# stattlab/azplugins

Hardware: AMD Instinct MI355X
Metric: particle-steps/sec, PerturbedLennardJones pair force (higher is better)
Workload: dtype f64

## Files before the change

### azplugins_amd/_lib.py

```python

import ctypes as C
import os

_HERE = os.path.dirname(os.path.abspath(__file__))
LIB_PATH = os.environ.get("AZP_LIB_PATH", os.path.join(_HERE, "libazp.so"))
CSRC = os.path.join(_HERE, "csrc")


class AzpError(RuntimeError):
    pass


class Box(C.Structure):
    _fields_ = [("L", C.c_double * 3), ("tilt", C.c_double * 3), ("periodic", C.c_int32 * 3), ("_pad", C.c_int32)]


class PairArgs(C.Structure):
    _fields_ = [
        ("d_force", C.c_void_p),
        ("d_virial", C.c_void_p),
        ("virial_pitch", C.c_uint64),
        ("N", C.c_uint32),
        ("n_max", C.c_uint32),
        ("d_pos", C.c_void_p),
# ... 607 lines not shown
    "azp_colloid_params_make": (None, [_D] * 4 + [_VP]),
    "azp_colloid_params_unpack": (None, [_VP] + [_PD] * 4),
    "azp_tpm_params_make": (None, [_D] * 5 + [C.c_int, _VP]),
    "azp_tpm_params_unpack": (None, [_VP] + [_PD] * 5 + [_PI]),
    "azp_dw_params_make": (None, [_D] * 4 + [_VP]),
    "azp_dw_params_unpack": (None, [_VP] + [_PD] * 4),
    "azp_quartic_params_make": (None, [_D] * 8 + [_VP]),
    "azp_quartic_params_unpack": (None, [_VP] + [_PD] * 8),
    "azp_table_pack": (C.c_int, [_D, _D, _VP, _VP, C.c_uint32, C.c_int, _VP]),
    "azp_pair_forces_table": (C.c_int, [C.POINTER(PairArgs), _VP, _VP]),
    "azp_pair_forces_planned_table": (C.c_int, [_VP, C.POINTER(PairArgs), _VP, _VP]),
    "azp_bond_forces_table": (C.c_int, [C.POINTER(BondArgs), _VP, _VP, _VP]),
    "azp_pair_forces_perturbed_lennard_jones": (C.c_int, [C.POINTER(PairArgs), _VP, _VP]),
    "azp_pair_forces_hertz": (C.c_int, [C.POINTER(PairArgs), _VP, _VP]),
    "azp_pair_forces_expanded_yukawa": (C.c_int, [C.POINTER(PairArgs), _VP, _VP]),
    "azp_pair_forces_colloid": (C.c_int, [C.POINTER(PairArgs), _VP, _VP]),
    "azp_pair_forces_dpd_conservative": (C.c_int, [C.POINTER(PairArgs), _VP, _VP]),
    "azp_pair_plan_create": (C.c_int, [C.POINTER(_VP)]),
    "azp_pair_plan_destroy": (None, [_VP]),
    "azp_pair_plan_build": (C.c_int, [_VP, C.POINTER(PairArgs), _VP]),
    "azp_pair_plan_build_from_cells": (C.c_int, [_VP, C.POINTER(NlistArgs), C.POINTER(PairArgs), _VP]),
    "azp_pair_plan_set_bank_order": (C.c_int, [_VP, C.c_int]),
    "azp_pair_plan_set_balance": (C.c_int, [_VP, C.c_int]),
    "azp_pair_plan_tile_stage": (C.c_int, [_VP, C.POINTER(C.c_uint32), C.c_uint32]),
    "azp_pair_plan_query": (C.c_int, [_VP, C.POINTER(PlanInfo)]),
    "azp_pair_plan_phase_chunks": (C.c_int, [_VP, C.POINTER(C.c_float)]),
    "azp_pair_plan_shells": (C.c_uint32, []),
    "azp_pair_plan_shells_for": (C.c_uint32, [_D, C.c_int, _D]),
    "azp_pair_plan_row_batches": (C.c_int, [_VP, C.POINTER(C.c_uint32), C.c_uint32, _PD]),
    "azp_sum_forces": (C.c_int, [C.c_uint32, C.c_uint32, C.POINTER(C.c_void_p), _VP, _VP]),
    "azp_pair_auto_plan_get_stats": (None, [C.POINTER(AutoPlanStats)]),
    "azp_pair_auto_plan_clear": (None, []),
    "azp_pair_forces_planned_perturbed_lennard_jones": (C.c_int, [_VP, C.POINTER(PairArgs), _VP, _VP]),
    "azp_pair_forces_planned_hertz": (C.c_int, [_VP, C.POINTER(PairArgs), _VP, _VP]),
    "azp_pair_forces_planned_expanded_yukawa": (C.c_int, [_VP, C.POINTER(PairArgs), _VP, _VP]),
    "azp_pair_forces_planned_colloid": (C.c_int, [_VP, C.POINTER(PairArgs), _VP, _VP]),
    "azp_pair_forces_planned_dpd_conservative": (C.c_int, [_VP, C.POINTER(PairArgs), _VP, _VP]),
    "azp_dpd_forces_general_weight": (C.c_int, [C.POINTER(DPDArgs), _VP, _VP]),
    "azp_aniso_forces_two_patch_morse": (C.c_int, [C.POINTER(AnisoArgs), _VP, _VP]),
    "azp_dpd_forces_planned_general_weight": (C.c_int, [_VP, C.POINTER(DPDArgs), _VP, _VP]),
    "azp_aniso_forces_planned_two_patch_morse": (C.c_int, [_VP, C.POINTER(AnisoArgs), _VP, _VP]),
    "azp_bond_forces_double_well": (C.c_int, [C.POINTER(BondArgs), _VP, _VP, _VP]),
    "azp_bond_forces_quartic": (C.c_int, [C.POINTER(BondArgs), _VP, _VP, _VP]),
    "azp_special_pair_lj_params_make": (None, [_D] * 3 + [_VP]),
    "azp_special_pair_lj_params_unpack": (None, [_VP] + [_PD] * 3),
    "azp_special_pair_forces_lj": (C.c_int, [C.POINTER(PairGroupArgs), _VP, _VP]),
# ... 171 lines not shown
class PairPlan:

    def __init__(self):
        self._h = _VP()
        check(lib().azp_pair_plan_create(C.byref(self._h)), "azp_pair_plan_create")

    def build(self, args, stream):
        check(lib().azp_pair_plan_build(self._h, C.byref(args), stream), "azp_pair_plan_build")

    def build_from_cells(self, cells, pair, stream):
        check(lib().azp_pair_plan_build_from_cells(self._h, C.byref(cells), C.byref(pair), stream), "azp_pair_plan_build_from_cells")

    def tile_stage(self):
        import numpy as np

        n = self.info()["n_tiles"]
        out = np.zeros(max(n, 1), dtype=np.uint32)
        m = lib().azp_pair_plan_tile_stage(self._h, out.ctypes.data_as(C.POINTER(C.c_uint32)), n)
        return out[:max(m, 0)]

    def set_balance(self, enabled):
        check(lib().azp_pair_plan_set_balance(self._h, int(bool(enabled))), "azp_pair_plan_set_balance")

    def set_bank_order(self, enabled):
        check(lib().azp_pair_plan_set_bank_order(self._h, int(bool(enabled))), "azp_pair_plan_set_bank_order")

    def info(self):
        i = PlanInfo()
        check(lib().azp_pair_plan_query(self._h, C.byref(i)), "azp_pair_plan_query")
        return {f[0]: getattr(i, f[0]) for f in PlanInfo._fields_ if f[0] != "_pad"}

    def phase_chunks(self):
        out = (C.c_float * 3)()
        check(lib().azp_pair_plan_phase_chunks(self._h, out), "azp_pair_plan_phase_chunks")
        return [float(x) for x in out]

    def row_batches(self):
        import numpy as np

        cols = int(lib().azp_pair_plan_shells()) + 1
        out = np.zeros(max(4 * self.info()["n_tiles"], 1) * cols, dtype=np.uint32)
        w = C.c_double(0.0)
        m = lib().azp_pair_plan_row_batches(self._h, out.ctypes.data_as(C.POINTER(C.c_uint32)), out.size, C.byref(w))
        if m < 0:
            check(m, "azp_pair_plan_row_batches")
        return out[:m].reshape(-1, cols), w.value
# ... 26 lines not shown
```

### azplugins_amd/csrc/pair_plan.hip

```cpp
#include <algorithm>
#include <vector>

#include "azp_device.hpp"
#include "pair_plan.hpp"

namespace azp
{
struct PlanKArgs
    {
    const double* pos;
    const uint32_t* n_neigh;
    const uint32_t* nlist;
    const uint64_t* head_list;
    const double* rcutsq;
    const double* rinnersq;
    uint32_t* slice_Kend;
    uint32_t* slice_Kphase;
    uint32_t n_slices;
    double r_list_max;
    double r_list_estimate;
    uint32_t bank_order;
    uint32_t* tile_nstage;
    uint64_t* tile_head;
    uint32_t* stage_idx;
// ... 447 lines not shown
        hipError_t e = hipFree(ptr);
        if (e != hipSuccess) return e;
        ptr = nullptr;
        }
    const size_t newcap = need + need / 8 + 64;
    hipError_t e = hipMalloc(reinterpret_cast<void**>(&ptr), newcap * sizeof(T));
    cap = (e == hipSuccess) ? newcap : 0;
    return e;
    }

void plan_free(PairPlan& p)
    {
    if (p.d_tile_nstage) (void)hipFree(p.d_tile_nstage);
    if (p.d_tile_head) (void)hipFree(p.d_tile_head);
    if (p.d_stage_idx) (void)hipFree(p.d_stage_idx);
    if (p.d_slice_K) (void)hipFree(p.d_slice_K);
    if (p.d_slice_Kend) (void)hipFree(p.d_slice_Kend);
    if (p.d_slice_Kphase) (void)hipFree(p.d_slice_Kphase);
    if (p.d_slice_head) (void)hipFree(p.d_slice_head);
    if (p.d_cnl) (void)hipFree(p.d_cnl);
    if (p.d_flags) (void)hipFree(p.d_flags);
    if (p.d_raw) (void)hipFree(p.d_raw);
    if (p.d_perm) (void)hipFree(p.d_perm);
    p = PairPlan();
    }

static size_t plan_lds_bytes(uint32_t hc, uint32_t stride)
    {
    const size_t shared_region = std::max<size_t>(4096 * 4, (size_t)stride * 16);
    return (size_t)hc * 4 + (size_t)hc * 2 + (size_t)PLAN_BUILD_WAVES * PLAN_ROWBUF * 2 + shared_region;
    }

template<int TPP, uint32_t HC> static hipError_t launch_plan_build(const PlanKArgs& k, uint32_t n_tiles, hipStream_t s)
    {
    const size_t lds = plan_lds_bytes(HC, k.stage_stride);
    auto kern = plan_build_kernel<TPP, HC>;
    if (lds + 18 * 1024 > 64 * 1024)
        {
        hipError_t e = hipFuncSetAttribute(reinterpret_cast<const void*>(kern),
                                           hipFuncAttributeMaxDynamicSharedMemorySize, (int)lds);
        if (e != hipSuccess)
            return e;
        }
    hipLaunchKernelGGL(kern, dim3(n_tiles), dim3(PLAN_BUILD_THREADS), lds, s, k);
    return hipGetLastError();
    }
// ... 21 lines not shown
        {                                      \
        hipError_t e_ = (expr);                \
        if (e_ != hipSuccess) return (int)e_;  \
        } while (0)

static int plan_build_tpp(PairPlan& p, const azp_pair_args& args, uint32_t tpp, hipStream_t s)
    {
    p.valid = false;
    p.invalid_reason = 0;
    p.tpp = tpp;
    p.tile = 256 / tpp;
    p.n_tiles = (args.N + p.tile - 1) / p.tile;
    p.n_slices = p.n_tiles * 4;

    size_t cap_heads_t = p.d_tile_head ? p.cap_tiles : 0, cap_heads_s = p.d_slice_head ? p.cap_slices : 0;
    AZP_HIP_TRY(ensure(p.d_tile_nstage, p.cap_tiles, p.n_tiles));
    AZP_HIP_TRY(ensure(p.d_tile_head, cap_heads_t, p.n_tiles));
    AZP_HIP_TRY(ensure(p.d_slice_K, p.cap_slices, p.n_slices));
    AZP_HIP_TRY(ensure(p.d_slice_Kend, p.cap_kend, (PLAN_SHELLS + 1) * (size_t)p.n_slices));
    AZP_HIP_TRY(ensure(p.d_slice_head, cap_heads_s, p.n_slices));
    AZP_HIP_TRY(ensure(p.d_slice_Kphase, p.cap_kphase, 2 * (size_t)p.n_slices));
    size_t cap_flags = p.d_flags ? 16 : 0;
    AZP_HIP_TRY(ensure(p.d_flags, cap_flags, 16));
    AZP_HIP_TRY(hipMemsetAsync(p.d_flags, 0, 8 * sizeof(uint32_t), s));

    PlanKArgs k;
    k.pos = args.d_pos;
    k.n_neigh = args.d_n_neigh;
    k.nlist = args.d_nlist;
    k.head_list = args.d_head_list;
    k.rcutsq = args.d_rcutsq;
    k.rinnersq = args.d_rinnersq;
    k.slice_Kend = p.d_slice_Kend;
    k.slice_Kphase = p.d_slice_Kphase;
    k.n_slices = p.n_slices;
    k.r_list_max = args.r_list_max;
    k.r_list_estimate = p.shell_hint_r_list;
    k.bank_order = p.bank_order ? 1u : 0u;
    k.tile_nstage = p.d_tile_nstage;
    k.tile_head = p.d_tile_head;
    k.stage_idx = nullptr;
    k.slice_K = p.d_slice_K;
    k.slice_head = p.d_slice_head;
    k.cnl = nullptr;
    k.flags = p.d_flags;
    k.box = make_box_dev(args.box);
// ... 109 lines not shown
    if (!plan)
        return;
    azp::PairPlan* p = reinterpret_cast<azp::PairPlan*>(plan);
    azp::plan_free(*p);
    delete p;
    }

extern "C" int azp_pair_plan_build(azp_pair_plan* plan, const azp_pair_args* args, void* stream)
    {
    if (!plan || !args || !args->d_pos || !args->d_n_neigh || !args->d_nlist || !args->d_head_list || !args->d_rcutsq
        || args->ntypes == 0)
        return AZP_ERROR_INVALID_ARGUMENT;
    return azp::plan_build(*reinterpret_cast<azp::PairPlan*>(plan), *args, static_cast<hipStream_t>(stream));
    }

extern "C" int azp_pair_plan_set_bank_order(azp_pair_plan* plan, int enabled)
    {
    if (!plan)
        return AZP_ERROR_INVALID_ARGUMENT;
    reinterpret_cast<azp::PairPlan*>(plan)->bank_order = enabled != 0;
    return AZP_SUCCESS;
    }

extern "C" int azp_pair_plan_set_balance(azp_pair_plan* plan, int enabled)
    {
    if (!plan)
        return AZP_ERROR_INVALID_ARGUMENT;
    reinterpret_cast<azp::PairPlan*>(plan)->balance = enabled != 0;
    return AZP_SUCCESS;
    }

extern "C" int azp_pair_plan_tile_stage(const azp_pair_plan* plan, uint32_t* out, uint32_t n)
    {
    if (!plan || !out)
        return AZP_ERROR_INVALID_ARGUMENT;
    const azp::PairPlan* p = reinterpret_cast<const azp::PairPlan*>(plan);
    const uint32_t m = std::min<uint32_t>(n, (uint32_t)p->h_tile_nstage.size());
    for (uint32_t t = 0; t < m; ++t)
        out[t] = p->h_tile_nstage[t];
    return (int)m;
    }

extern "C" int azp_pair_plan_query(const azp_pair_plan* plan, azp_pair_plan_info* info)
    {
    if (!plan || !info)
        return AZP_ERROR_INVALID_ARGUMENT;
// ... 75 lines not shown
```

### azplugins_amd/csrc/pair_plan.hpp

```cpp
#pragma once
#include <cmath>
#include <vector>

#include <hip/hip_runtime.h>
#include <stdint.h>

#include "../../include/azp.h"

namespace azp
{
constexpr uint32_t PLAN_HASH_CAP = 8192;
constexpr uint32_t PLAN_MAX_STAGE = 2559;
constexpr uint32_t PLAN_EMPTY = 0xFFFFFFFFu;
constexpr uint32_t PLAN_BITMAP_WORDS = 80;
constexpr uint32_t PLAN_ROWBUF = 512;
constexpr double PLAN_FAR = 1.0e30;
constexpr uint32_t PLAN_SHELLS = 16;
constexpr uint32_t PLAN_SHELL_CLASSES = 13;
constexpr uint32_t PLAN_CLASSES = PLAN_SHELL_CLASSES + 3;
static_assert(PLAN_CLASSES <= 16 && PLAN_SHELL_CLASSES <= PLAN_SHELLS, "an entry's class is kept in 4 bits");
constexpr uint32_t PLAN_CLS_CORE = 0;
constexpr uint32_t PLAN_CLS_SURE = 1;
constexpr uint32_t PLAN_CLS_NEAR = 2;
constexpr uint32_t PLAN_CLS_SHELL0 = 3;
// ... 28 lines not shown
    float core_r = 0.f;
    float sure_r = 0.f;
    double shell_width = 0.0;
    float max_listed_r = 0.f;
    double shell_hint_r_list = 0.0;
    uint64_t* d_slice_head = nullptr;
    uint4* d_cnl = nullptr;
    uint32_t* d_flags = nullptr;
    size_t cap_tiles = 0, cap_slices = 0, cap_stage = 0, cap_cnl = 0, cap_kend = 0;
    uint64_t builds = 0;
    bool from_cells = false;
    uint32_t row_cap = 0;
    uint32_t max_row = 0;
    uint16_t* d_raw = nullptr;
    uint32_t max_member_cells = 0;
    size_t cap_raw = 0;
    bool balance = false;
    bool balanced = false;
    uint8_t* d_perm = nullptr;
    size_t cap_perm = 0;
    bool bank_order = true;
    uint32_t stage_stride_hint = 0;
    std::vector<uint32_t> h_tile_nstage;
    };

inline uint32_t plan_shells_for_width(double shell_width, bool has_bound, double bound)
    {
    if (!has_bound || !(bound >= 0.0))
        return PLAN_SHELLS;
    if (bound == 0.0)
        return 0;
    if (!(shell_width > 0.0))
        return PLAN_SHELLS;
    const double n = std::ceil(2.0 * bound * (1.0 + 1e-12) / shell_width);
    return n >= (double)PLAN_SHELLS ? PLAN_SHELLS : (uint32_t)n;
    }

inline uint32_t plan_shells_for(const PairPlan& plan, const azp_pair_args& args)
    {
    return plan_shells_for_width(plan.shell_width, args.has_displacement_bound != 0, args.displacement_bound);
    }

int plan_build(PairPlan& p, const azp_pair_args& args, hipStream_t s);
int plan_build_from_cells(PairPlan& p, const azp_nlist_args& cells, const azp_pair_args& pair, hipStream_t s);
void plan_free(PairPlan& p);

inline uint32_t plan_cap_for(uint32_t max_stage)
    {
    const uint32_t need = max_stage + 1;
    return need <= 1024 ? 1024 : (need <= 1536 ? 1536 : (need <= 1664 ? 1664 : (need <= 2048 ? 2048 : 2560)));
    }

}
```

### azplugins_amd/csrc/pair_plan_cells.hip

```cpp
#include <algorithm>
#include <cstdio>
#include <cstdlib>
#include <vector>

#include "azp_device.hpp"
#include "pair_plan.hpp"

namespace azp
{
#ifdef AZP_PLAN_CELLS_PROFILE
#define PC_PROFILE_AND(x) && (x)
#else
#define PC_PROFILE_AND(x)
#endif

constexpr uint32_t PC_THREADS = 256;
constexpr uint32_t PC_BATCH = 1024;
constexpr uint32_t PC_MAXCAND = 8192;
constexpr uint32_t PC_MAXCELLS = 512;
constexpr uint32_t PC_MAXMC = 128;
constexpr uint32_t PC_RUNS = 18;
constexpr uint32_t PC_SETA = 512, PC_SETB = 1024;
constexpr uint32_t PC_ROWMAX = 512;
constexpr uint32_t PC_EMPTY = 0xffffffffu;
// ... 1044 lines not shown
    if (c.N == 0)
        return AZP_SUCCESS;
    if (c.box.tilt[0] != 0.0 || c.box.tilt[1] != 0.0 || c.box.tilt[2] != 0.0 || c.fractional_cells || c.ntypes > 255)
        {
        p.invalid_reason = 6;
        return AZP_SUCCESS;
        }
    uint32_t row_cap = c.row_capacity ? c.row_capacity : 160u;
    row_cap = std::min<uint32_t>((row_cap + 7u) & ~7u, PC_ROWMAX - 8u);
    p.tpp = 1;
    p.tile = 256;
    p.n_tiles = (c.N + 255u) / 256u;
    p.n_slices = p.n_tiles * 4;
    p.row_cap = row_cap;
    size_t cap_heads_t = p.d_tile_head ? p.cap_tiles : 0, cap_heads_s = p.d_slice_head ? p.cap_slices : 0;
    AZP_HIP_TRY(ensure_buf(p.d_tile_nstage, p.cap_tiles, p.n_tiles));
    AZP_HIP_TRY(ensure_buf(p.d_tile_head, cap_heads_t, p.n_tiles));
    AZP_HIP_TRY(ensure_buf(p.d_slice_K, p.cap_slices, p.n_slices));
    AZP_HIP_TRY(ensure_buf(p.d_slice_Kend, p.cap_kend, (PLAN_SHELLS + 1) * (size_t)p.n_slices));
    AZP_HIP_TRY(ensure_buf(p.d_slice_head, cap_heads_s, p.n_slices));
    AZP_HIP_TRY(ensure_buf(p.d_slice_Kphase, p.cap_kphase, 2 * (size_t)p.n_slices));
    size_t cap_flags = p.d_flags ? 16 : 0;
    AZP_HIP_TRY(ensure_buf(p.d_flags, cap_flags, 16));
    p.total_chunks = (uint64_t)p.n_slices * (row_cap / 8u);
    AZP_HIP_TRY(ensure_buf(p.d_cnl, p.cap_cnl, (size_t)p.total_chunks * 64));
    AZP_HIP_TRY(ensure_buf(p.d_raw, p.cap_raw, (size_t)p.n_tiles * 256u * row_cap));
    p.balanced = false;
    if (p.balance)
        AZP_HIP_TRY(ensure_buf(p.d_perm, p.cap_perm, (size_t)p.n_tiles * 256u));

    PlanCellsKArgs k;
    k.pos = c.d_pos;
    k.rlistsq = c.d_rlistsq;
    k.rcutsq = pa.d_rcutsq;
    k.rinnersq = pa.d_rinnersq;
    k.cell_of = c.d_cell_of;
    k.order = c.d_order;
    k.cell_start = c.d_cell_start;
    k.n_excl = c.d_n_excl;
    k.excl = c.d_excl;
    k.excl_pitch = c.excl_pitch;
    k.n_neigh = c.d_n_neigh;
    k.raw = p.d_raw;
    k.tile_nstage = p.d_tile_nstage;
    k.tile_head = p.d_tile_head;
    k.slice_K = p.d_slice_K;
// ... 114 lines not shown
```

### azplugins_amd/csrc/pair_tiled.hpp

```cpp
#pragma once

#include <type_traits>

#include "pair_kernel.hpp"
#include "pair_plan.hpp"

#ifndef AZP_TILED_WAVES_PER_SIMD
#define AZP_TILED_WAVES_PER_SIMD 4
#endif

namespace azp
{
#ifdef AZP_TIMELINE
extern __device__ unsigned long long g_timeline[8 * 4 * 16384];
#endif

struct TileDyn
    {
    uint32_t n_shells;
    uint32_t stale;
    };

struct TiledKArgs
    {
    PairKArgs p;
    const uint32_t* tile_nstage;
    const uint64_t* tile_head;
    const uint32_t* stage_idx;
    const uint32_t* slice_Kend;
    uint32_t n_shells;
    const uint64_t* slice_head;
    const uint4* cnl;
    const uint8_t* perm;
    const TileDyn* dyn;
    const uint32_t* dflag;
    const unsigned long long* dbits;
    const float* disp;
    double shell_w;
    double shell_winv;
    double bound_extra;
    const uint32_t* slice_Kphase;
    double core_reach_sq;
    uint32_t fast_stage;
    };

__device__ __forceinline__ float wave_max_nonneg(float v)
    {
#pragma unroll
    for (int off = 32; off > 0; off >>= 1)
        v = fmaxf(v, __shfl_xor(v, off, 64));
    return v;
    }

__device__ __forceinline__ uint32_t tile_shells_for(double b, double shell_winv)
    {
    if (!(b >= 0.0))
        return PLAN_SHELLS;
    if (b == 0.0)
        return 0u;
    if (!(shell_winv > 0.0))
        return PLAN_SHELLS;
    const double n = ceil(2.0 * b * (1.0 + 1e-9) * shell_winv);
    return n >= (double)PLAN_SHELLS ? PLAN_SHELLS : (uint32_t)n;
    }

template<class T> __device__ __forceinline__ T load_uniform(const T* p)
    {
    return *(const __attribute__((address_space(4))) T*)p;
    }

__device__ __forceinline__ double4 load_scalar4_o32(const double* base, uint32_t idx)
    {
    const char* p = reinterpret_cast<const char*>(base) + (idx << 5);
    const double2 a = *reinterpret_cast<const double2*>(p);
    const double2 b = *reinterpret_cast<const double2*>(p + 16);
    return make_double4(a.x, a.y, b.x, b.y);
    }
__device__ __forceinline__ double3 load_scalar3_of4_o32(const double* base, uint32_t idx)
    {
    const char* p = reinterpret_cast<const char*>(base) + (idx << 5);
    const double2 a = *reinterpret_cast<const double2*>(p);
    const double z = *reinterpret_cast<const double*>(p + 16);
    return make_double3(a.x, a.y, z);
    }

#define AZP_TILE_STRIDE(CAP) ((CAP) + 1)

constexpr int TILE_BATCH = 4;

struct TileBatch
    {
// ... 243 lines not shown
        constexpr int ROUNDS = (CAP + 255) / 256;
        uint32_t sj[ROUNDS];
#pragma unroll
        for (int r = 0; r < ROUNDS; ++r)
            {
            const uint32_t sidx = (uint32_t)r * 256u + tid;
            sj[r] = (sidx < n_stage) ? stage[sidx] : first;
            }
        __builtin_amdgcn_sched_barrier(0);
        const uint32_t idx = first + (a.perm ? (uint32_t)member : wave * 64u + lane);
        const bool active = idx < a.p.end;
        if (((a.dyn != nullptr) & (w_stale != 0u)) | ((a.dflag != nullptr) & (w_flag != 0u)))
            return;
#ifdef AZP_TIMELINE
        __builtin_amdgcn_s_waitcnt(0);
        tl_tb = __builtin_amdgcn_s_memrealtime();
#endif
        uint32_t n_shells = a.dyn ? min(w_shells, PLAN_SHELLS) : a.n_shells;
        if (a.dbits)
            n_shells = tile_shells_for(to_uniform(sqrt(__longlong_as_double((long long)w_bits)) + a.bound_extra), a.shell_winv);
        uint32_t Kb = load_uniform(a.slice_Kend + ((PLAN_SHELLS + 1) * slice + min(n_shells, PLAN_SHELLS)));
        uint32_t Kcore = load_uniform(a.core_reach_sq > 0.0 ? a.slice_Kphase + slice : spare);

        const Coeff c0 = to_uniform(E::prepare(params[0], load_uniform(a.p.rcutsq), a.p.shift_mode == AZP_SHIFT_SHIFT));
        const double rcutsq_max = c0.rcutsq;
        if (!(a.core_reach_sq > 0.0 && c0.wca_rsq <= a.core_reach_sq))
            Kcore = 0xffffffffu;
        asm volatile("" ::"s"(c.x), "s"(c.y), "s"(c.z), "s"(slice_head), "s"(Kb), "s"(Kcore), "s"(a.fast_stage), "s"(a.p.pos));
        __builtin_amdgcn_sched_barrier(0);
#ifdef AZP_TIMELINE
        tl_ta = __builtin_amdgcn_s_memrealtime();
#endif
        if (tid == 0)
            {
            s_x[0] = PLAN_FAR; s_y[0] = PLAN_FAR; s_z[0] = PLAN_FAR;
            }

        double3 pi = make_double3(0.0, 0.0, 0.0);
        bool lane_wide = false;
        float dmax = 0.f;
        const uint32_t me = active ? idx : first;
        if (a.disp)
            {
            dmax = a.disp[me];
#pragma unroll
            for (int r = 0; r < ROUNDS; ++r)
                dmax = fmaxf(dmax, a.disp[sj[r]]);
            }
        double sxv[ROUNDS], syv[ROUNDS], szv[ROUNDS];
        if (a.fast_stage)
            {
// ... 73 lines not shown
                    if (a.p.box.px) x = __builtin_fma(-a.p.box.Lx, rint((x - c.x) * a.p.box.Lxinv), x);
                    if (a.p.box.py) y = __builtin_fma(-a.p.box.Ly, rint((y - c.y) * a.p.box.Lyinv), y);
                    if (a.p.box.pz) z = __builtin_fma(-a.p.box.Lz, rint((z - c.z) * a.p.box.Lzinv), z);
                    const double rx = no_hint ? 0.25 * a.p.box.Lx : a.p.r_list_max, ry = no_hint ? 0.25 * a.p.box.Ly : a.p.r_list_max,
                                 rz = no_hint ? 0.25 * a.p.box.Lz : a.p.r_list_max;
                    lane_wide = lane_wide || (a.p.box.px && fabs(x - c.x) + rx >= 0.5 * a.p.box.Lx)
                                || (a.p.box.py && fabs(y - c.y) + ry >= 0.5 * a.p.box.Ly)
                                || (a.p.box.pz && fabs(z - c.z) + rz >= 0.5 * a.p.box.Lz);
                    }
                pi = make_double3(x, y, z);
                }
            }
#ifdef AZP_TIMELINE
        __builtin_amdgcn_s_waitcnt(0);
        tl_td = __builtin_amdgcn_s_memrealtime();
#endif
        __shared__ float s_dmax[4];
        if (a.disp)
            {
            dmax = wave_max_nonneg(dmax);
            if (lane == 0)
                s_dmax[wave] = dmax;
            }
        const bool wide = __syncthreads_or(lane_wide);
        __builtin_amdgcn_s_setprio(0);
#ifdef AZP_TIMELINE
        const unsigned long long tl_t1 = __builtin_amdgcn_s_memrealtime();
#endif
        if (a.disp)
            {
            const float d4 = fmaxf(fmaxf(s_dmax[0], s_dmax[1]), fmaxf(s_dmax[2], s_dmax[3]));
            const uint32_t tile_shells = tile_shells_for(to_uniform((double)d4 + a.bound_extra), a.shell_winv);
            Kb = to_uniform(a.slice_Kend[(PLAN_SHELLS + 1) * slice + min(tile_shells, PLAN_SHELLS)]);
            }
        const char* __restrict__ slice_base = reinterpret_cast<const char*>(a.cnl + slice_head * 64ull);
        const uint32_t lane_off = lane * 16u;

        double fx = 0.0, fy = 0.0, fz = 0.0, pe = 0.0;
        double v[6] = {0.0, 0.0, 0.0, 0.0, 0.0, 0.0};
        uint32_t n_core = 0, n_in = 0;
        double es[2] = {0.0, 0.0};
        const char* bx = reinterpret_cast<const char*>(s_x);
        if (wide)
            tiled_loop<E, 1, CAP, VIRIAL, true, false, true>(a, bx, nullptr, nullptr, nullptr, c0, 0.0, rcutsq_max, slice_base, lane_off, Kb, pi, 0,
                                                             fx, fy, fz, pe, v, n_core, n_in, es);
        else
            tiled_loop_phases<E, 1, CAP, VIRIAL>(a, bx, c0, rcutsq_max, slice_base, lane_off, Kb, Kcore, pi, 0, fx, fy, fz, pe, v, n_core,
                                                 n_in, es);
        pe = E::finish_split(c0, pe, es[0], es[1], n_core, n_in);

#ifdef AZP_TIMELINE
// ... 281 lines not shown
    k.cnl = plan.d_cnl;
    k.slice_Kphase = plan.d_slice_Kphase;
    k.core_reach_sq = plan_core_reach_sq(plan, args, k);
    k.fast_stage = (!k.p.box.triclinic && k.p.box.px && k.p.box.py && k.p.box.pz && k.p.r_list_max > 0.0 && args.n_max < (1u << 27)) ? 1u : 0u;
    const uint32_t t0 = k.p.first / tb, t1 = (k.p.end + tb - 1) / tb;
    k.p.first = t0 * tb;
    k.p.end = (t1 * tb < args.N) ? t1 * tb : args.N;
    k.p.nblocks_padded = (t1 - t0 + 7u) & ~7u;
    return k;
    }

inline uint32_t plan_launch_cap(const PairPlan& plan, const azp_pair_args& args, uint32_t tb)
    {
    if (args.range_count == 0 || plan.h_tile_nstage.empty())
        return plan.cap;
    const uint32_t end = (args.range_first + args.range_count < args.N) ? args.range_first + args.range_count : args.N;
    const uint32_t t0 = args.range_first / tb, t1 = (end + tb - 1) / tb;
    uint32_t most = 0;
    for (uint32_t t = t0; t < t1 && t < plan.n_tiles; ++t)
        most = plan.h_tile_nstage[t] > most ? plan.h_tile_nstage[t] : most;
    return plan_cap_for(most);
    }

template<class E, int TPP, int CAP, bool VIRIAL, bool SINGLE>
int launch_tiled_instance(const PairPlan& plan, const azp_pair_args& args, const typename E::Params* d_params,
                          hipStream_t stream, const TileDyn* dyn)
    {
    const TiledKArgs k = make_tiled_kargs(plan, args, dyn, plan.tile);
    size_t lds = (size_t)AZP_TILE_STRIDE(CAP) * 24 + (SINGLE ? 0 : (size_t)CAP * 4 + 8);
    if (!SINGLE)
        lds += (sizeof(typename E::Coeff) + sizeof(double)) * (size_t)args.ntypes * args.ntypes;
    if (args.shift_mode == AZP_SHIFT_XPLOR)
        return launch_dyn_lds(pair_forces_tiled_kernel<E, TPP, CAP, VIRIAL, SINGLE, true>, k.p.nblocks_padded, 256, TPP, lds, stream, k, d_params);
    return launch_dyn_lds(pair_forces_tiled_kernel<E, TPP, CAP, VIRIAL, SINGLE, false>, k.p.nblocks_padded, 256, TPP, lds, stream, k, d_params);
    }

template<class E, int TPP, bool VIRIAL, bool SINGLE>
int launch_tiled_cap(const PairPlan& plan, const azp_pair_args& args, const typename E::Params* d_params, hipStream_t s, const TileDyn* dyn)
    {
    const uint32_t cap = plan_launch_cap(plan, args, plan.tile);
    switch (cap)
        {
    case 1024: return launch_tiled_instance<E, TPP, 1024, VIRIAL, SINGLE>(plan, args, d_params, s, dyn);
    case 1536: return launch_tiled_instance<E, TPP, 1536, VIRIAL, SINGLE>(plan, args, d_params, s, dyn);
    case 1664: return launch_tiled_instance<E, TPP, 1664, VIRIAL, SINGLE>(plan, args, d_params, s, dyn);
    case 2048: return launch_tiled_instance<E, TPP, 2048, VIRIAL, SINGLE>(plan, args, d_params, s, dyn);
    case 2560: return launch_tiled_instance<E, TPP, 2560, VIRIAL, SINGLE>(plan, args, d_params, s, dyn);
    default: return AZP_ERROR_INVALID_ARGUMENT;
        }
    }

// ... 24 lines not shown
```

### azplugins_amd/pair.py

```python

import ctypes as C

import numpy as np

from . import _lib
from .force import Force, ScalarTypeParameter, TableTypeParameter, TypeParameter

_SHIFT = {"none": 0, "shift": 1, "xplor": 2}


class Pair(Force):

    _cpp_class_name = None
    _entry = None
    _planned_entry = None
    _plan_balance = False
    _schema = {}
    _param_doubles = 4
    _accepted_modes = ("none", "shift", "xplor")
    _halo_fields = ("pos",)

    def __init__(self, nlist, default_r_cut=None, default_r_on=0.0, mode="none"):
        super().__init__()
        if mode not in self._accepted_modes:
            raise ValueError("mode must be one of %s, got %r" % (self._accepted_modes, mode))
        self.nlist = nlist
        self._mode = mode
        self.params = TypeParameter("params", self._schema, 2, self._mark_dirty, self._readback)
        self.r_cut = ScalarTypeParameter("r_cut", default_r_cut, self._r_cut_changed)
        self.r_on = ScalarTypeParameter("r_on", default_r_on, self._mark_dirty)
        self.threads_per_particle = 0
        self.block_size = 0
        self.use_plan = True
        self.use_displacement_bound = True
        self.use_local_displacement = False
        self.plan_bank_order = None
        self.use_fused_plan = True
        self.use_speculative_launch = True
        self._plan = None
        self._plan_builds = None
        self._plan_valid = False
        self._plan_ids = None
        self._plan_disp0 = None
        self._calls_since_plan = None
        self._spec_cache = None
        self._fused_refused_types = None
        self._tables = None
        self._cpp = None
        self._cpp_synced = False
        nlist.add_consumer(self)

    @property
    def mode(self):
        return self._mode

    @mode.setter
    def mode(self, m):
        if m not in self._accepted_modes:
            raise ValueError("mode must be one of %s, got %r" % (self._accepted_modes, m))
        self._mode = m
        self._mark_dirty()

    def _mark_dirty(self):
        self._tables = None
        self._cpp_synced = False
        self._plan_builds = None

    def _r_cut_changed(self):
        self._mark_dirty()
        self.nlist.consumers_changed()

    def _pack(self, d):
        raise NotImplementedError

    def _unpack(self, raw):
        raise NotImplementedError

    def _readback(self, key):
        if not self._attached or key not in self.params._data:
            return None
        self._sync_cpp()
        return dict(self._cpp.getParams(*key))

# ... 31 lines not shown

    def _attach(self, sim):
        super()._attach(sim)
        self._tables = None
        self._cpp = None
        self._cpp_synced = False

    def _build_tables(self):
        import torch

        types = self._state.types
        T = len(types)
        for a in types:
            for b in types:
                if self.params.get_raw((a, b)) is None:
                    raise _lib.AzpError("%s.params[(%r, %r)] is not set" % (type(self).__name__, a, b))
        self._sync_cpp()
        raw = np.frombuffer(self._cpp.params_bytes(), dtype=np.float64).reshape(T * T, -1).copy()
        assert raw.shape[1] == self._param_doubles
        rc = np.asarray(self._cpp.rcutsq())
        ro = np.asarray(self._cpp.ronsq())
        dev = self._state.device
        self._spec_cache = None
        self._tables = dict(
            params=torch.from_numpy(raw).to(dev), rcutsq=torch.from_numpy(rc).to(dev), ronsq=torch.from_numpy(ro).to(dev)
        )
        inner = np.zeros(T * T)
        for i, a in enumerate(types):
            for j, b in enumerate(types):
                inner[i * T + j] = self._inner_radius(self.params.get_raw((a, b))) ** 2
        if inner.any():
            self._tables["rinnersq"] = torch.from_numpy(inner).to(dev)

    def _inner_radius(self, d):
        return 0.0

    def takes_plan_from_cells(self):
        st = self._state
        refused = st is not None and self._fused_refused_types == len(st.types)
        return bool(self.use_plan and self._planned_entry and self.threads_per_particle in (0, 1) and self.use_fused_plan
                    and not refused)

    def _pair_args(self, particle_range=None):
        st, nl = self._state, self.nlist
        a = _lib.PairArgs()
        a.d_force = self._force.data_ptr()
# ... 67 lines not shown
            self._list_mode_for_launch(True)
            a = self._pair_args()
            a.has_displacement_bound, a.displacement_bound, a.d_displacement = 0, 0.0, None
            a.displacement_bound_extra = self._plan_disp0
            self._spec_cache = (sig, boxc, a)
        a.d_stale_flag, a.d_displacement_sq_bits = token["flag_ptr"], token["bits_ptr"]
        entry, args = self._prepare_launch(_lib.raw_stream(st.device), timestep, a=a)
        _lib.check(getattr(_lib.lib(), entry)(*args), entry)
        if nl.end_check(token):
            return False
        return True

    def _prepare_launch(self, stream, timestep, particle_range=None, a=None):
        planned = self.use_plan and self._planned_entry is not None
        if a is None:
            self._list_mode_for_launch(planned)
            a = self._pair_args(particle_range)
            if planned:
                self._plan_step(a, stream)
        args, params = C.byref(self._wrap_args(a, timestep)), self._tables["params"].data_ptr()
        if not planned:
            return self._entry, (args, params, stream)
        self._calls_since_plan += 1
        return self._planned_entry, (self._plan.handle, args, params, stream)

    def _list_mode_for_launch(self, planned):
        nl = self.nlist
        if nl.fused_active and not (planned and self.use_fused_plan):
            nl.leave_fused_mode()
        if self._plan_ids is not None and not nl.fused_active:
            self._plan_ids = self._plan_builds = None

    def _plan_step(self, a, stream):
        key = self._plan_key()
        if self._plan_builds == key:
            return
        if self._plan is None:
            self._plan = _lib.PairPlan()
        nl = self.nlist
        first, count = a.range_first, a.range_count
        a.range_first = a.range_count = 0
        if nl.fused_active:
            self._plan.set_balance(self._plan_balance)
            info = nl.compile_plan(self._plan, a, stream)
            self._plan_valid = bool(info["valid"])
            if info["valid"]:
                self._plan_ids = (info["list_id"], info["head_id"])
                a.d_nlist, a.d_head_list = self._plan_ids
                self._plan_builds = key
                self._calls_since_plan = 0
                self._plan_disp0 = 0.0
                b = nl.displacement_bound(self._state)
                known = b is not None and self.use_displacement_bound
                a.has_displacement_bound, a.displacement_bound = (1, b) if known else (0, 0.0)
                a.displacement_bound_extra = 0.0
            else:
                a.d_nlist, a.d_head_list, a.size_nlist = nl.nlist.data_ptr(), nl.head_list.data_ptr(), nl.size
        if self._plan_builds != key:
            calls = self._calls_since_plan
            self._plan.set_bank_order((calls is None or calls >= 50) if self.plan_bank_order is None else self.plan_bank_order)
            self._calls_since_plan = 0
# ... 212 lines not shown
                    continue
                rows = _lib.table_pack(d["r_min"], rc, d["U"], d["F"], closed=False)
                if rows is None:
                    raise _lib.AzpError("%s.params[(%r, %r)]: needs 0 <= r_min < r_cut and finite U, F of equal length "
                                        "(r_min = %g, r_cut = %g)" % (name, a, b, d["r_min"], rc))
                packed[(a, b)] = (first, rows)
                first += len(rows)
        all_rows = np.concatenate([rows for _, rows in packed.values()] + [np.zeros((1, 4))])
        d_rows = torch.from_numpy(all_rows).to(dev)
        assert d_rows.data_ptr() % 32 == 0
        entries, rc2, ro2 = [], np.zeros(T * T), np.zeros(T * T)
        for i, a in enumerate(types):
            for j, b in enumerate(types):
                key = (a, b) if i <= j else (b, a)
                rc2[i * T + j] = self.r_cut[key] ** 2
                ro2[i * T + j] = self.r_on[key] ** 2
                if key in packed:
                    at, rows = packed[key]
                    entries.append((self.params.get_raw(key)["r_min"], self.r_cut[key], d_rows.data_ptr() + 32 * at, len(rows)))
                else:
                    entries.append((0.0, 0.0, 0, 0))
        self._spec_cache = None
        self._plan_builds = None
        self._tables = dict(params=torch.from_numpy(_lib.table_params_rows(entries)).to(dev), rcutsq=torch.from_numpy(rc2).to(dev),
                            ronsq=torch.from_numpy(ro2).to(dev), rows=d_rows)


__all__ = ["Colloid", "DPDGeneralWeight", "DPDConservativeGeneralWeight", "ExpandedYukawa", "Hertz",
           "PerturbedLennardJones", "Table", "TwoPatchMorse"]
```

### include/azp.h

```cpp
#ifndef AZP_H_
#define AZP_H_

#include <stddef.h>
#include <stdint.h>

#ifdef __cplusplus
extern "C" {
#endif

#define AZP_VERSION_MAJOR 0
#define AZP_VERSION_MINOR 2

typedef enum azp_status
    {
    AZP_SUCCESS = 0,
    AZP_ERROR_INVALID_ARGUMENT = -1,
    AZP_ERROR_TOO_MANY_TYPES = -2,
    AZP_ERROR_NO_DEVICE = -3,
    AZP_ERROR_TOO_MANY_BINS = -4
    } azp_status;

typedef enum azp_shift_mode
    {
    AZP_SHIFT_NONE = 0,
// ... 97 lines not shown
    int32_t invalid_reason;
    uint32_t threads_per_particle;
    uint32_t tile_size;
    uint32_t lds_slots;
    uint32_t n_tiles;
    uint32_t max_stage;
    uint32_t max_row;
    uint64_t total_stage;
    uint64_t compiled_bytes;
    uint64_t builds;
    int32_t from_cells;
    uint32_t row_capacity;
    uint64_t list_id, head_id;
    int32_t balanced;
    float core_radius;
    float sure_radius;
    uint32_t max_member_cells;
    } azp_pair_plan_info;

int azp_pair_plan_create(azp_pair_plan** out);
void azp_pair_plan_destroy(azp_pair_plan* plan);
int azp_pair_plan_build(azp_pair_plan* plan, const azp_pair_args* args, void* stream);
int azp_pair_plan_set_balance(azp_pair_plan* plan, int enabled);
int azp_pair_plan_tile_stage(const azp_pair_plan* plan, uint32_t* out, uint32_t n);
int azp_pair_plan_set_bank_order(azp_pair_plan* plan, int enabled);
int azp_pair_plan_query(const azp_pair_plan* plan, azp_pair_plan_info* info);
int azp_pair_plan_phase_chunks(const azp_pair_plan* plan, float out[3]);
uint32_t azp_pair_plan_shells(void);
uint32_t azp_pair_plan_shells_for(double shell_width, int has_bound, double bound);
int azp_pair_plan_row_batches(const azp_pair_plan* plan, uint32_t* out, uint32_t n, double* shell_width);

typedef struct azp_auto_plan_stats
    {
    uint64_t calls;
    uint64_t compiles;
    uint64_t reuses;
    uint64_t generic_fallbacks;
    } azp_auto_plan_stats;
void azp_pair_auto_plan_get_stats(azp_auto_plan_stats* out);
void azp_pair_auto_plan_clear(void);

int azp_pair_forces_planned_perturbed_lennard_jones(azp_pair_plan* plan, const azp_pair_args* args,
                                                    const azp_plj_params* d_params, void* stream);
int azp_pair_forces_planned_hertz(azp_pair_plan* plan, const azp_pair_args* args, const azp_hertz_params* d_params,
                                  void* stream);
int azp_pair_forces_planned_expanded_yukawa(azp_pair_plan* plan, const azp_pair_args* args,
// ... 740 lines not shown
```

Before: 9.419 billion.

## Precompute single-type pair coefficients in a cached device table keyed by parameter generation

Moves the per-block E::prepare call for the single-type tiled kernel into a one-thread kernel that writes the Coeff struct to a plan-owned buffer. The buffer is refilled only when the parameter generation, pointers, shift mode or stream change, and the tiled kernel loads it with scalar uniform loads. It also replaces __syncthreads_or with per-wave __any plus an LDS reduction. This is meant to remove redundant coefficient math (divisions/powers) from every block's prologue, at the cost of generation bookkeeping and possible staleness if parameters change without a generation bump.

```diff
diff --git a/azplugins_amd/_lib.py b/azplugins_amd/_lib.py
--- a/azplugins_amd/_lib.py
+++ b/azplugins_amd/_lib.py
@@ -653,6 +653,7 @@
     "azp_pair_plan_build_from_cells": (C.c_int, [_VP, C.POINTER(NlistArgs), C.POINTER(PairArgs), _VP]),
     "azp_pair_plan_set_bank_order": (C.c_int, [_VP, C.c_int]),
     "azp_pair_plan_set_balance": (C.c_int, [_VP, C.c_int]),
+    "azp_pair_plan_set_param_generation": (C.c_int, [_VP, C.c_uint64]),
     "azp_pair_plan_tile_stage": (C.c_int, [_VP, C.POINTER(C.c_uint32), C.c_uint32]),
     "azp_pair_plan_query": (C.c_int, [_VP, C.POINTER(PlanInfo)]),
     "azp_pair_plan_phase_chunks": (C.c_int, [_VP, C.POINTER(C.c_float)]),
@@ -870,6 +871,9 @@
     def set_balance(self, enabled):
         check(lib().azp_pair_plan_set_balance(self._h, int(bool(enabled))), "azp_pair_plan_set_balance")
 
+    def set_param_generation(self, generation):
+        check(lib().azp_pair_plan_set_param_generation(self._h, int(generation)), "azp_pair_plan_set_param_generation")
+
     def set_bank_order(self, enabled):
         check(lib().azp_pair_plan_set_bank_order(self._h, int(bool(enabled))), "azp_pair_plan_set_bank_order")
 
diff --git a/azplugins_amd/csrc/pair_plan.hip b/azplugins_amd/csrc/pair_plan.hip
--- a/azplugins_amd/csrc/pair_plan.hip
+++ b/azplugins_amd/csrc/pair_plan.hip
@@ -493,6 +493,7 @@
     if (p.d_flags) (void)hipFree(p.d_flags);
     if (p.d_raw) (void)hipFree(p.d_raw);
     if (p.d_perm) (void)hipFree(p.d_perm);
+    if (p.d_coeff) (void)hipFree(p.d_coeff);
     p = PairPlan();
     }
 
@@ -560,6 +561,7 @@
     AZP_HIP_TRY(ensure(p.d_slice_Kphase, p.cap_kphase, 2 * (size_t)p.n_slices));
     size_t cap_flags = p.d_flags ? 16 : 0;
     AZP_HIP_TRY(ensure(p.d_flags, cap_flags, 16));
+    AZP_HIP_TRY(plan_ensure_coeff(p));
     AZP_HIP_TRY(hipMemsetAsync(p.d_flags, 0, 8 * sizeof(uint32_t), s));
 
     PlanKArgs k;
@@ -715,6 +717,14 @@
     return AZP_SUCCESS;
     }
 
+extern "C" int azp_pair_plan_set_param_generation(azp_pair_plan* plan, uint64_t generation)
+    {
+    if (!plan)
+        return AZP_ERROR_INVALID_ARGUMENT;
+    reinterpret_cast<azp::PairPlan*>(plan)->param_generation = generation;
+    return AZP_SUCCESS;
+    }
+
 extern "C" int azp_pair_plan_set_balance(azp_pair_plan* plan, int enabled)
     {
     if (!plan)
diff --git a/azplugins_amd/csrc/pair_plan.hpp b/azplugins_amd/csrc/pair_plan.hpp
--- a/azplugins_amd/csrc/pair_plan.hpp
+++ b/azplugins_amd/csrc/pair_plan.hpp
@@ -74,6 +74,20 @@
     bool bank_order = true;
     uint32_t stage_stride_hint = 0;
     std::vector<uint32_t> h_tile_nstage;
+    struct CoeffKey
+        {
+        uint64_t generation = 0;
+        const void* d_params = nullptr;
+        const void* d_rcutsq = nullptr;
+        int shift_mode = -1;
+        const void* evaluator = nullptr;
+        hipStream_t stream = nullptr;
+        bool valid = false;
+        };
+    static constexpr size_t COEFF_TABLE_BYTES = 256;
+    void* d_coeff = nullptr;
+    uint64_t param_generation = 0;
+    mutable CoeffKey coeff_key;
     };
 
 inline uint32_t plan_shells_for_width(double shell_width, bool has_bound, double bound)
@@ -97,6 +111,14 @@
 int plan_build_from_cells(PairPlan& p, const azp_nlist_args& cells, const azp_pair_args& pair, hipStream_t s);
 void plan_free(PairPlan& p);
 
+inline hipError_t plan_ensure_coeff(PairPlan& p)
+    {
+    if (p.d_coeff)
+        return hipSuccess;
+    p.coeff_key = PairPlan::CoeffKey();
+    return hipMalloc(&p.d_coeff, PairPlan::COEFF_TABLE_BYTES);
+    }
+
 inline uint32_t plan_cap_for(uint32_t max_stage)
     {
     const uint32_t need = max_stage + 1;
diff --git a/azplugins_amd/csrc/pair_plan_cells.hip b/azplugins_amd/csrc/pair_plan_cells.hip
--- a/azplugins_amd/csrc/pair_plan_cells.hip
+++ b/azplugins_amd/csrc/pair_plan_cells.hip
@@ -1090,6 +1090,7 @@
     AZP_HIP_TRY(ensure_buf(p.d_slice_Kphase, p.cap_kphase, 2 * (size_t)p.n_slices));
     size_t cap_flags = p.d_flags ? 16 : 0;
     AZP_HIP_TRY(ensure_buf(p.d_flags, cap_flags, 16));
+    AZP_HIP_TRY(plan_ensure_coeff(p));
     p.total_chunks = (uint64_t)p.n_slices * (row_cap / 8u);
     AZP_HIP_TRY(ensure_buf(p.d_cnl, p.cap_cnl, (size_t)p.total_chunks * 64));
     AZP_HIP_TRY(ensure_buf(p.d_raw, p.cap_raw, (size_t)p.n_tiles * 256u * row_cap));
diff --git a/azplugins_amd/csrc/pair_tiled.hpp b/azplugins_amd/csrc/pair_tiled.hpp
--- a/azplugins_amd/csrc/pair_tiled.hpp
+++ b/azplugins_amd/csrc/pair_tiled.hpp
@@ -42,6 +42,7 @@
     const uint32_t* slice_Kphase;
     double core_reach_sq;
     uint32_t fast_stage;
+    const void* coeff;
     };
 
 __device__ __forceinline__ float wave_max_nonneg(float v)
@@ -67,6 +68,18 @@
 template<class T> __device__ __forceinline__ T load_uniform(const T* p)
     {
     return *(const __attribute__((address_space(4))) T*)p;
+    }
+
+template<class T> __device__ __forceinline__ T load_uniform_struct(const T* p)
+    {
+    static_assert(sizeof(T) % sizeof(double) == 0 && alignof(T) >= alignof(double), "64-bit words");
+    T v;
+    const double* src = reinterpret_cast<const double*>(p);
+    double* dst = reinterpret_cast<double*>(&v);
+#pragma unroll
+    for (int w = 0; w < (int)(sizeof(T) / sizeof(double)); ++w)
+        dst[w] = load_uniform(src + w);
+    return v;
     }
 
 __device__ __forceinline__ double4 load_scalar4_o32(const double* base, uint32_t idx)
@@ -356,11 +369,18 @@
         uint32_t Kb = load_uniform(a.slice_Kend + ((PLAN_SHELLS + 1) * slice + min(n_shells, PLAN_SHELLS)));
         uint32_t Kcore = load_uniform(a.core_reach_sq > 0.0 ? a.slice_Kphase + slice : spare);
 
-        const Coeff c0 = to_uniform(E::prepare(params[0], load_uniform(a.p.rcutsq), a.p.shift_mode == AZP_SHIFT_SHIFT));
+        const Coeff c0 = load_uniform_struct(static_cast<const Coeff*>(a.coeff));
         const double rcutsq_max = c0.rcutsq;
         if (!(a.core_reach_sq > 0.0 && c0.wca_rsq <= a.core_reach_sq))
             Kcore = 0xffffffffu;
         asm volatile("" ::"s"(c.x), "s"(c.y), "s"(c.z), "s"(slice_head), "s"(Kb), "s"(Kcore), "s"(a.fast_stage), "s"(a.p.pos));
+        {
+        static_assert(sizeof(Coeff) % sizeof(double) == 0, "the coefficients are pinned as 64-bit words");
+        const double* cw = reinterpret_cast<const double*>(&c0);
+#pragma unroll
+        for (int w = 0; w < (int)(sizeof(Coeff) / sizeof(double)); ++w)
+            asm volatile("" ::"s"(cw[w]));
+        }
         __builtin_amdgcn_sched_barrier(0);
 #ifdef AZP_TIMELINE
         tl_ta = __builtin_amdgcn_s_memrealtime();
@@ -480,11 +500,17 @@
             if (lane == 0)
                 s_dmax[wave] = dmax;
             }
-        const bool wide = __syncthreads_or(lane_wide);
+        __shared__ __attribute__((aligned(16))) uint32_t s_wide[4];
+        const bool wave_wide = __any(lane_wide);
+        if (lane == 0)
+            s_wide[wave] = wave_wide ? 1u : 0u;
+        __syncthreads();
         __builtin_amdgcn_s_setprio(0);
 #ifdef AZP_TIMELINE
         const unsigned long long tl_t1 = __builtin_amdgcn_s_memrealtime();
 #endif
+        const uint4 wides = *reinterpret_cast<const uint4*>(s_wide);
+        const bool wide = to_uniform(wides.x | wides.y | wides.z | wides.w) != 0u;
         if (a.disp)
             {
             const float d4 = fmaxf(fmaxf(s_dmax[0], s_dmax[1]), fmaxf(s_dmax[2], s_dmax[3]));
@@ -812,11 +838,69 @@
     return plan_cap_for(most);
     }
 
+template<class E>
+__global__ void __launch_bounds__(64) tile_coeff_kernel(const typename E::Params* __restrict__ params, const double* __restrict__ rcutsq,
+                                                        int shift_mode, typename E::Coeff* __restrict__ out)
+    {
+    if (threadIdx.x == 0)
+        *out = E::prepare(params[0], rcutsq[0], shift_mode == AZP_SHIFT_SHIFT);
+    }
+
+template<class E>
+int ensure_coeff_table(const PairPlan& plan, const azp_pair_args& args, const typename E::Params* d_params, hipStream_t stream)
+    {
+    static_assert(sizeof(typename E::Coeff) <= PairPlan::COEFF_TABLE_BYTES, "the plan's coefficient buffer holds one Coeff");
+    if (!plan.d_coeff)
+        return AZP_ERROR_INVALID_ARGUMENT;
+    auto kern = tile_coeff_kernel<E>;
+    PairPlan::CoeffKey key;
+    key.generation = plan.param_generation;
+    key.d_params = d_params;
+    key.d_rcutsq = args.d_rcutsq;
+    key.shift_mode = args.shift_mode;
+    key.evaluator = reinterpret_cast<const void*>(kern);
+    key.stream = stream;
+    key.valid = true;
+    const PairPlan::CoeffKey& have = plan.coeff_key;
+    if (key.generation != 0 && have.valid && have.generation == key.generation && have.d_params == key.d_params
+        && have.d_rcutsq == key.d_rcutsq && have.shift_mode == key.shift_mode && have.evaluator == key.evaluator
+        && have.stream == key.stream)
+        return AZP_SUCCESS;
+    hipLaunchKernelGGL(kern, dim3(1), dim3(64), 0, stream, d_params, args.d_rcutsq, args.shift_mode,
+                       static_cast<typename E::Coeff*>(plan.d_coeff));
+    const hipError_t e = hipGetLastError();
+    if (e != hipSuccess)
+        return (int)e;
+    if (key.generation != 0)
+        {
+        hipStreamCaptureStatus cap = hipStreamCaptureStatusNone;
+        if (hipStreamIsCapturing(stream, &cap) != hipSuccess)
+            {
+            (void)hipGetLastError();
+            key.valid = false;
+            }
+        else if (cap != hipStreamCaptureStatusNone)
+            key.valid = false;
+        }
+    plan.coeff_key = key;
+    return AZP_SUCCESS;
+    }
+
 template<class E, int TPP, int CAP, bool VIRIAL, bool SINGLE>
 int launch_tiled_instance(const PairPlan& plan, const azp_pair_args& args, const typename E::Params* d_params,
                           hipStream_t stream, const TileDyn* dyn)
     {
-    const TiledKArgs k = make_tiled_kargs(plan, args, dyn, plan.tile);
+    TiledKArgs k = make_tiled_kargs(plan, args, dyn, plan.tile);
+    if constexpr (TPP == 1 && SINGLE && E::kSplitEnergy)
+        {
+        if (args.shift_mode != AZP_SHIFT_XPLOR)
+            {
+            const int rc = ensure_coeff_table<E>(plan, args, d_params, stream);
+            if (rc != AZP_SUCCESS)
+                return rc;
+            k.coeff = plan.d_coeff;
+            }
+        }
     size_t lds = (size_t)AZP_TILE_STRIDE(CAP) * 24 + (SINGLE ? 0 : (size_t)CAP * 4 + 8);
     if (!SINGLE)
         lds += (sizeof(typename E::Coeff) + sizeof(double)) * (size_t)args.ntypes * args.ntypes;
diff --git a/azplugins_amd/pair.py b/azplugins_amd/pair.py
--- a/azplugins_amd/pair.py
+++ b/azplugins_amd/pair.py
@@ -46,6 +46,8 @@
         self._spec_cache = None
         self._fused_refused_types = None
         self._tables = None
+        self._param_gen = 1
+        self._plan_gen_sent = None
         self._cpp = None
         self._cpp_synced = False
         nlist.add_consumer(self)
@@ -59,6 +61,7 @@
         if m not in self._accepted_modes:
             raise ValueError("mode must be one of %s, got %r" % (self._accepted_modes, m))
         self._mode = m
+        self._param_gen += 1
         self._mark_dirty()
 
     def _mark_dirty(self):
@@ -136,6 +139,7 @@
         ro = np.asarray(self._cpp.ronsq())
         dev = self._state.device
         self._spec_cache = None
+        self._param_gen += 1
         self._tables = dict(
             params=torch.from_numpy(raw).to(dev), rcutsq=torch.from_numpy(rc).to(dev), ronsq=torch.from_numpy(ro).to(dev)
         )
@@ -249,6 +253,9 @@
         if not planned:
             return self._entry, (args, params, stream)
         self._calls_since_plan += 1
+        if self._plan_gen_sent != self._param_gen:
+            self._plan.set_param_generation(self._param_gen)
+            self._plan_gen_sent = self._param_gen
         return self._planned_entry, (self._plan.handle, args, params, stream)
 
     def _list_mode_for_launch(self, planned):
@@ -264,6 +271,7 @@
             return
         if self._plan is None:
             self._plan = _lib.PairPlan()
+            self._plan_gen_sent = None
         nl = self.nlist
         first, count = a.range_first, a.range_count
         a.range_first = a.range_count = 0
@@ -522,6 +530,7 @@
                     entries.append((0.0, 0.0, 0, 0))
         self._spec_cache = None
         self._plan_builds = None
+        self._param_gen += 1
         self._tables = dict(params=torch.from_numpy(_lib.table_params_rows(entries)).to(dev), rcutsq=torch.from_numpy(rc2).to(dev),
                             ronsq=torch.from_numpy(ro2).to(dev), rows=d_rows)
 
diff --git a/include/azp.h b/include/azp.h
--- a/include/azp.h
+++ b/include/azp.h
@@ -143,6 +143,7 @@
 void azp_pair_plan_destroy(azp_pair_plan* plan);
 int azp_pair_plan_build(azp_pair_plan* plan, const azp_pair_args* args, void* stream);
 int azp_pair_plan_set_balance(azp_pair_plan* plan, int enabled);
+int azp_pair_plan_set_param_generation(azp_pair_plan* plan, uint64_t generation);
 int azp_pair_plan_tile_stage(const azp_pair_plan* plan, uint32_t* out, uint32_t n);
 int azp_pair_plan_set_bank_order(azp_pair_plan* plan, int enabled);
 int azp_pair_plan_query(const azp_pair_plan* plan, azp_pair_plan_info* info);
```

After: 9.490 billion, median of 6. No clear change (+0.8%).
